# VodLM/vod

Hardware: AMD Instinct MI355X
Metric: queries/sec brute-force top-k (10Mx768 fp16) (higher is better)
Workload: dtype f16; 1 GPU; 10000000 sections x 768 f16, batch 1024 queries, top-100, exact brute force; rows_per_gpu=10000000, parallelism=single GPU, engine=ranks, recovery_passes=0

## Files before the change

### include/vodhip.h

```cpp
#ifndef VODHIP_H
#define VODHIP_H

#include <stdint.h>

#ifdef __cplusplus
extern "C" {
#endif

#define VODHIP_VERSION 1

enum { VODHIP_F16 = 0, VODHIP_BF16 = 1, VODHIP_F32 = 2 };
#define VODHIP_EXACT_F32 0x100
#define VODHIP_L2 0x200
enum { VODHIP_HOST = 0, VODHIP_DEVICE = 1 };

typedef struct vodhip_index vodhip_index_t;

const char* vodhip_last_error(void);
int vodhip_version(void);

int vodhip_index_create(int device, int64_t dim, int store_dtype ,
                        int64_t capacity_rows, vodhip_index_t** out);
int vodhip_index_destroy(vodhip_index_t* index);

// ... 47 lines not shown

#define VODHIP_POSTERIOR_GROUP_ROWS 16384
#define VODHIP_POSTERIOR_TEMP_BYTES (256ll << 20)
int vodhip_index_posterior_mean(vodhip_index_t* index, const void* queries, int q_dtype, int64_t nq, float beta,
                                const int32_t* q_labels_dev , int n_per_query,
                                float* out_max , float* out_log_rel ,
                                float* out_mean , void* stream);

#define VODHIP_SAMPLE_SLACK_TILES 2
int vodhip_index_sample_posterior(vodhip_index_t* index, const void* queries, int q_dtype, int64_t nq, int k, float beta, uint64_t seed,
                                  int64_t query_offset, int64_t id_base, const int32_t* q_labels_dev ,
                                  int n_per_query, float* out_max , float* out_log_rel ,
                                  int64_t* out_ids , float* out_scores, float* out_log_p,
                                  float* out_log_weight , float* out_keys , void* stream);

#define VODHIP_RANK_MAX_LISTED 64
int vodhip_index_count_above(vodhip_index_t* index, const void* queries, int q_dtype, int64_t nq, const float* thresholds_dev,
                             const int64_t* tie_ids_dev , int64_t m, int64_t id_base,
                             const int32_t* q_labels_dev , int n_per_query,
                             int64_t* out_counts , void* stream);
int vodhip_index_rank_ids(vodhip_index_t* index, const void* queries, int q_dtype, int64_t nq, const int64_t* ids_dev, int64_t m,
                          int64_t id_base, const int32_t* q_labels_dev , int n_per_query,
                          int64_t* out_ranks , float* out_scores , void* stream);
int vodhip_index_scan_score_ids(vodhip_index_t* index, const void* queries, int q_dtype, int64_t nq, const int64_t* ids_dev, int64_t m,
                                int64_t id_base, const int32_t* q_labels_dev , int n_per_query,
                                float* out_scores , int32_t* out_rows , void* stream);

int vodhip_index_set_row_labels(vodhip_index_t* index, const int32_t* labels, int64_t n_rows, int location, void* stream);
int vodhip_index_set_query_labels(vodhip_index_t* index, const int32_t* q_labels_dev, int n_per_query);

int vodhip_index_set_param(vodhip_index_t* index, const char* key, int64_t value);
int vodhip_debug_schedule(int64_t ntotal, int k, int64_t nq, int64_t cand_cap, int64_t dense_rows, int64_t sample_div,
                          int64_t growth_x100, int tile, int recovery_pass, int n_cu, int64_t* out, int max_stages);
int vodhip_index_get_stat(const vodhip_index_t* index, const char* key, int64_t* out);
int vodhip_debug_l2_split(float c, int dtype, uint16_t terms[3], float consts[3]);
int vodhip_debug_tile_order(int64_t ntotal, int64_t* perm_mul, int64_t* perm_mod);
int vodhip_debug_read_probe(int which, int64_t* out, int n);

int vodhip_merge_topk(const float* scores, const int64_t* ids, int n_shards, int64_t nq, int k,
                      int k_out, float* out_scores, int64_t* out_ids, void* stream);
int vodhip_merge_topk_strided(const float* scores, int64_t shard_stride_scores, const int64_t* ids,
                              int64_t shard_stride_ids, int n_shards, int64_t nq, int k, int k_out,
                              float* out_scores, int64_t* out_ids, void* stream);

typedef struct vodhip_node_index vodhip_node_index_t;
int vodhip_node_index_create(int n_devices, const int* devices, int64_t dim, int store_dtype, int64_t capacity_rows,
                             vodhip_node_index_t** out);
int vodhip_node_index_destroy(vodhip_node_index_t* index);
int vodhip_node_index_add(vodhip_node_index_t* index, const void* rows, int64_t n_rows, int src_dtype);
int vodhip_node_index_reset(vodhip_node_index_t* index);
int vodhip_node_index_ntotal(const vodhip_node_index_t* index, int64_t* out);
int vodhip_node_index_n_shards(const vodhip_node_index_t* index);
int vodhip_node_index_shard(vodhip_node_index_t* index, int g, vodhip_index_t** shard, int64_t* id_base, int* device);
int vodhip_node_index_set_param(vodhip_node_index_t* index, const char* key, int64_t value);
int vodhip_node_index_peer_access(const vodhip_node_index_t* index, int* out, int n);
int vodhip_node_index_set_row_labels(vodhip_node_index_t* index, const int32_t* labels, int64_t n_rows);
int vodhip_node_index_set_query_labels(vodhip_node_index_t* index, const int32_t* q_labels, int n_per_query, int location);
int vodhip_node_index_search(vodhip_node_index_t* index, const void* queries, int q_dtype, int64_t nq, int k, int location,
                             float* out_scores, int64_t* out_ids, void* stream);
int vodhip_node_index_search_async(vodhip_node_index_t* index, const void* queries, int q_dtype, int64_t nq, int k, int location,
                                   float* out_scores, int64_t* out_ids, void* stream);
int vodhip_node_index_search_finish(vodhip_node_index_t* index);
int vodhip_node_index_score_ids(vodhip_node_index_t* index, const void* queries, int q_dtype, int64_t nq, const int64_t* ids, int64_t m,
                                const int32_t* q_labels, int n_per_query, int location, float* out_scores, void* stream);
int vodhip_node_index_search_ids(vodhip_node_index_t* index, const void* queries, int q_dtype, int64_t nq, const int64_t* ids, int64_t m,
                                 int k, const int32_t* q_labels, int n_per_query, int location, float* out_scores, int64_t* out_ids,
// ... 248 lines not shown
```

### vod_amd/_native.py

```python
from __future__ import annotations

import ctypes
import pathlib
import threading

_LIB_NAME = "libvodhip.so"
_lock = threading.Lock()
_lib: ctypes.CDLL | None = None

F16, BF16, F32 = 0, 1, 2
EXACT_F32 = 0x100
L2 = 0x200
METRICS = {"inner_product": 0, "l2": L2}


def metric_flag(metric: str) -> int:
    if metric not in METRICS:
        raise ValueError(f"metric must be one of {sorted(METRICS)}, got {metric!r}")
    return METRICS[metric]
HOST, DEVICE = 0, 1
MAX_K = 2048
MAX_LISTED = 8192
MAX_ENGINES = 4

# ... 17 lines not shown
SIGNATURES: dict[str, tuple] = {
    "vodhip_last_error": (_c.c_char_p, []),
    "vodhip_version": (_i32, []),
    "vodhip_index_create": (_i32, [_i32, _i64, _i32, _i64, _c.POINTER(_vp)]),
    "vodhip_index_destroy": (_i32, [_vp]),
    "vodhip_index_add": (_i32, [_vp, _vp, _i64, _i32, _i32, _vp]),
    "vodhip_index_reset": (_i32, [_vp]),
    "vodhip_index_ntotal": (_i32, [_vp, _c.POINTER(_i64)]),
    "vodhip_index_dim": (_i32, [_vp, _c.POINTER(_i64)]),
    "vodhip_index_capacity": (_i32, [_vp, _c.POINTER(_i64)]),
    "vodhip_index_data": (_i32, [_vp, _c.POINTER(_vp), _c.POINTER(_i64), _c.POINTER(_i32)]),
    "vodhip_index_get_rows": (_i32, [_vp, _i64, _i64, _vp, _i32, _vp]),
    "vodhip_index_data_f32": (_i32, [_vp, _c.POINTER(_vp), _c.POINTER(_i64)]),
    "vodhip_index_get_rows_f32": (_i32, [_vp, _i64, _i64, _vp, _i32, _vp]),
    "vodhip_index_search": (_i32, [_vp, _vp, _i32, _i64, _i32, _i64, _vp, _vp, _vp]),
    "vodhip_index_search_async": (_i32, [_vp, _vp, _i32, _i64, _i32, _i64, _vp, _vp, _vp]),
    "vodhip_index_search_finish": (_i32, [_vp, _vp]),
    "vodhip_index_score_ids": (_i32, [_vp, _vp, _i32, _i64, _vp, _i64, _i64, _vp, _i32, _vp, _vp]),
    "vodhip_index_search_ids": (_i32, [_vp, _vp, _i32, _i64, _vp, _i64, _i32, _i64, _vp, _i32, _vp, _vp, _vp]),
    "vodhip_index_sum_ids": (_i32, [_vp, _vp, _vp, _i64, _i64, _i64, _vp, _i32, _vp, _vp]),
    "vodhip_index_log_partition": (_i32, [_vp, _vp, _i32, _i64, _c.c_float, _vp, _i32, _vp, _vp, _vp]),
    "vodhip_index_posterior_stats": (_i32, [_vp, _vp, _i32, _i64, _c.c_float, _vp, _i32, _vp, _vp, _vp, _vp, _vp]),
    "vodhip_index_posterior_divergence": (_i32, [_vp, _vp, _vp, _i32, _i64, _c.c_float, _c.c_float, _vp, _i32] + [_vp] * 8 + [_vp]),
    "vodhip_index_posterior_mean": (_i32, [_vp, _vp, _i32, _i64, _c.c_float, _vp, _i32, _vp, _vp, _vp, _vp]),
    "vodhip_index_count_above": (_i32, [_vp, _vp, _i32, _i64, _vp, _vp, _i64, _i64, _vp, _i32, _vp, _vp]),
    "vodhip_index_rank_ids": (_i32, [_vp, _vp, _i32, _i64, _vp, _i64, _i64, _vp, _i32, _vp, _vp, _vp]),
    "vodhip_index_scan_score_ids": (_i32, [_vp, _vp, _i32, _i64, _vp, _i64, _i64, _vp, _i32, _vp, _vp, _vp]),
    "vodhip_index_sample_posterior": (
        _i32, [_vp, _vp, _i32, _i64, _i32, _c.c_float, _c.c_uint64, _i64, _i64, _vp, _i32, _vp, _vp, _vp, _vp, _vp, _vp, _vp, _vp]),
    "vodhip_index_set_row_labels": (_i32, [_vp, _vp, _i64, _i32, _vp]),
    "vodhip_index_set_query_labels": (_i32, [_vp, _vp, _i32]),
    "vodhip_index_set_param": (_i32, [_vp, _c.c_char_p, _i64]),
    "vodhip_debug_schedule": (_i32, [_i64, _i32, _i64, _i64, _i64, _i64, _i64, _i32, _i32, _i32, _c.POINTER(_i64), _i32]),
    "vodhip_index_get_stat": (_i32, [_vp, _c.c_char_p, _c.POINTER(_i64)]),
    "vodhip_debug_l2_split": (_i32, [_c.c_float, _i32, _c.POINTER(_c.c_uint16), _c.POINTER(_c.c_float)]),
    "vodhip_debug_tile_order": (_i32, [_i64, _c.POINTER(_i64), _c.POINTER(_i64)]),
    "vodhip_debug_read_probe": (_i32, [_i32, _c.POINTER(_i64), _i32]),
    "vodhip_node_index_create": (_i32, [_i32, _c.POINTER(_i32), _i64, _i32, _i64, _c.POINTER(_vp)]),
    "vodhip_node_index_destroy": (_i32, [_vp]),
    "vodhip_node_index_add": (_i32, [_vp, _vp, _i64, _i32]),
    "vodhip_node_index_reset": (_i32, [_vp]),
    "vodhip_node_index_ntotal": (_i32, [_vp, _c.POINTER(_i64)]),
    "vodhip_node_index_n_shards": (_i32, [_vp]),
    "vodhip_node_index_shard": (_i32, [_vp, _i32, _c.POINTER(_vp), _c.POINTER(_i64), _c.POINTER(_i32)]),
    "vodhip_node_index_set_param": (_i32, [_vp, _c.c_char_p, _i64]),
    "vodhip_node_index_get_stat": (_i32, [_vp, _c.c_char_p, _c.POINTER(_i64)]),
    "vodhip_node_index_peer_access": (_i32, [_vp, _c.POINTER(_i32), _i32]),
    "vodhip_node_index_set_row_labels": (_i32, [_vp, _vp, _i64]),
    "vodhip_node_index_set_query_labels": (_i32, [_vp, _vp, _i32, _i32]),
    "vodhip_node_index_search": (_i32, [_vp, _vp, _i32, _i64, _i32, _i32, _vp, _vp, _vp]),
    "vodhip_node_index_search_async": (_i32, [_vp, _vp, _i32, _i64, _i32, _i32, _vp, _vp, _vp]),
    "vodhip_node_index_search_finish": (_i32, [_vp]),
    "vodhip_node_index_score_ids": (_i32, [_vp, _vp, _i32, _i64, _vp, _i64, _vp, _i32, _i32, _vp, _vp]),
    "vodhip_node_index_search_ids": (_i32, [_vp, _vp, _i32, _i64, _vp, _i64, _i32, _vp, _i32, _i32, _vp, _vp, _vp]),
    "vodhip_node_index_sum_ids": (_i32, [_vp, _vp, _vp, _i64, _i64, _vp, _i32, _i32, _vp, _vp]),
    "vodhip_node_index_log_partition": (_i32, [_vp, _vp, _i32, _i64, _c.c_float, _vp, _i32, _vp, _vp]),
    "vodhip_node_index_posterior_stats": (_i32, [_vp, _vp, _i32, _i64, _c.c_float, _vp, _i32, _vp, _vp, _vp, _vp]),
    "vodhip_node_index_posterior_divergence": (_i32, [_vp, _vp, _vp, _i32, _i64, _c.c_float, _c.c_float, _vp, _i32] + [_vp] * 8),
    "vodhip_node_index_posterior_mean": (_i32, [_vp, _vp, _i32, _i64, _c.c_float, _vp, _i32, _vp, _vp, _vp]),
    "vodhip_node_index_rank_ids": (_i32, [_vp, _vp, _i32, _i64, _vp, _i64, _vp, _i32, _vp, _vp]),
    "vodhip_node_index_count_above": (_i32, [_vp, _vp, _i32, _i64, _vp, _vp, _i64, _vp, _i32, _vp]),
    "vodhip_node_index_sample_posterior": (
        _i32, [_vp, _vp, _i32, _i64, _i32, _c.c_float, _c.c_uint64, _i64, _vp, _i32, _vp, _vp, _vp, _vp, _vp, _vp, _vp]),
    "vodhip_merge_topk": (_i32, [_vp, _vp, _i32, _i64, _i32, _i32, _vp, _vp, _vp]),
    "vodhip_merge_topk_strided": (_i32, [_vp, _i64, _vp, _i64, _i32, _i64, _i32, _i32, _vp, _vp, _vp]),
    "vodhip_merge_hybrid": (
# ... 172 lines not shown
```

### vod_amd/csrc/kernels_mips_8phase.hip

```cpp
#include <hip/hip_runtime.h>

#include <type_traits>

#include "mips_common.h"

namespace vodhip {

namespace {
constexpr int P8_HALF = 128 * 128;
constexpr int P8_OPERANDS = 8 * P8_HALF;
constexpr int P8_WL_CAP = 256;
constexpr int P8_WL_FLUSH = 176;
constexpr int P8_TRANSPOSE_MAX_LANES = 2;
constexpr int P8_XPOSE = 8 * 2 * 32 * 4;
constexpr int P8_DRAIN_RECORDS = 112;
constexpr int P8_SC1 = 16;
static_assert(P8_DRAIN_RECORDS % 8 == 0 && P8_DRAIN_RECORDS * 132 + 256 <= P8_OPERANDS / 8, "drain staging");
constexpr int P8_LDS = P8_OPERANDS + 8 * P8_WL_CAP * 12 + P8_XPOSE;
static_assert(P8_LDS <= 160 * 1024, "LDS budget");
}

template <int DT, bool SUBSET, bool KEEPB0, int LEAD = 7>
__global__ __launch_bounds__(512, 2) void mips_filter8ph_kernel(
    const uint16_t* __restrict__ X, const uint16_t* __restrict__ Q, int dim_pad, int row_begin, int row_end, int n_xtiles,
    int n_qtiles, int nq, const float* __restrict__ thr_s, const key_t64* __restrict__ thr_key, key_t64* __restrict__ cand,
    unsigned int* __restrict__ cnt, int cap, unsigned int* __restrict__ overflow, FilterExtra ex, float* __restrict__ ring, int ring_cap) {
    constexpr int BM = 256, BN = 256, WN = 4, NWAVES = 8, TM = 128, TN = 64, MB = TM / 16, NB16 = TN / 16, ROW_BYTES = 128;
    extern __shared__ __attribute__((aligned(16))) char smem[];
    const int bid = blockIdx.x;
    const int xcd = bid & 7, jj = bid >> 3;
    const int qt = jj % n_qtiles;
    const int xt0 = (jj / n_qtiles) * 8 + xcd;
    const int xt_step = (int)gridDim.x / n_qtiles;
    if (xt0 >= n_xtiles) return;
    const int n_my = (n_xtiles - 1 - xt0) / xt_step + 1;
    const int tid = threadIdx.x;
    const int lane = tid & 63;
    const int wave = __builtin_amdgcn_readfirstlane(tid >> 6);
    const int wm = wave / WN, wn = wave % WN;
    const int q0 = qt * BN;
    const int nk = dim_pad / 64;
    const size_t row_stride = (size_t)dim_pad * 2;

    const int st_row = lane >> 3, st_slot = lane & 7;
    int super_cur = ex.perm_mod > 0 ? filter_tile_row0(ex, row_begin, xt0, BM) / BM : 0;
    int super_epi = super_cur;
    const int perm_inc = ex.perm_mod > 0 ? (int)(((unsigned long long)xt_step * (unsigned long long)ex.perm_mul) % (unsigned long long)ex.perm_mod) : 0;
    const char* a_src[2];
    const char* b_src[2];
#pragma unroll
// ... 54 lines not shown
                        a_src[0] += step;
                        a_src[1] += step;
                    } else {
                        s_active = false;
                    }
                }
            }
        }
    };
    using K0 = std::integral_constant<int, 0>;
    using K1 = std::integral_constant<int, 1>;
    using K2 = std::integral_constant<int, 2>;
    using K3 = std::integral_constant<int, 3>;

    const int fr = lane & 15, fq = lane >> 4;
    const int swz = (fr >> 1) & 7;

    float thr[NB16];
#pragma unroll
    for (int j = 0; j < NB16; ++j) {
        const int q = q0 + wn * TN + j * 16 + fr;
        thr[j] = q < nq ? thr_s[q] : __builtin_inff();
    }
#pragma unroll
    for (int j = 0; j < NB16; ++j) asm volatile("" : "+v"(thr[j]));
    wait_vmcnt<0>();

    WaveSurvivorList<P8_WL_CAP, SUBSET> wl(smem + P8_OPERANDS, NWAVES, wave);
    const SurvivorOut out{thr_key, cand, cnt, cap, overflow, ex};
    auto wl_append = [&](bool p, key_t64 key, int q) { if (wl.append(p, key, q, out)) wait_vmcnt<0>(); };
    auto wl_flush = [&]() { wl.flush(out); wait_vmcnt<0>(); };
    float* const xpose = (float*)(smem + P8_OPERANDS + NWAVES * P8_WL_CAP * 12) + wave * 64;
    const size_t ring_wave = (size_t)bid * NWAVES + wave;
    float* const ring_w = ring + ring_wave * ring_cap * 32;
    unsigned* const ring_meta = (unsigned*)(ring + (size_t)gridDim.x * NWAVES * ring_cap * 32) + ring_wave * ring_cap;
    int ring_n = 0;
    int ring_fallbacks = 0;

    f32x4 acc[MB][NB16];
    u32x4 fa[4], fb[2], fa1[4], fb1[2];
    u32x4 fc[2], fc1[2];
#ifdef P8_KNOBS
    const bool knob_no_stagger = (ex.flags & (1 << 8)) != 0, knob_no_prio = (ex.flags & (2 << 8)) != 0;
#else
    constexpr bool knob_no_stagger = false, knob_no_prio = false;
#endif

    auto read_a = [&](const char* half) {
        const char* base = half + (wm * 64 + fr) * ROW_BYTES;
        const int s0 = ((0 + fq) ^ swz) << 4, s1 = ((4 + fq) ^ swz) << 4;
#pragma unroll
        for (int i = 0; i < 4; ++i) {
            fa[i] = *(const u32x4*)(base + i * 16 * ROW_BYTES + s0);
            fa1[i] = *(const u32x4*)(base + i * 16 * ROW_BYTES + s1);
        }
    };
    auto read_b = [&](const char* half) {
        const char* base = half + (wn * 32 + fr) * ROW_BYTES;
        const int s0 = ((0 + fq) ^ swz) << 4, s1 = ((4 + fq) ^ swz) << 4;
#pragma unroll
        for (int j = 0; j < 2; ++j) {
            fb[j] = *(const u32x4*)(base + j * 16 * ROW_BYTES + s0);
            fb1[j] = *(const u32x4*)(base + j * 16 * ROW_BYTES + s1);
        }
    };
    auto read_b1 = [&](const char* half) {
        const char* base = half + (wn * 32 + fr) * ROW_BYTES;
        const int s0 = ((0 + fq) ^ swz) << 4, s1 = ((4 + fq) ^ swz) << 4;
// ... 53 lines not shown
        for (int j = 0; j < NB16; ++j) {
            mj[j] = vmax3(acc[0][j][0], acc[0][j][1], acc[0][j][2]);
            mj[j] = fmaxf_raw(mj[j], acc[0][j][3]);
        }
#pragma unroll
        for (int i = 1; i < MB; ++i)
#pragma unroll
            for (int j = 0; j < NB16; ++j) {
                mj[j] = vmax3(mj[j], acc[i][j][0], acc[i][j][1]);
                mj[j] = vmax3(mj[j], acc[i][j][2], acc[i][j][3]);
            }
#ifdef P8_ABL_NO_EMIT
#pragma unroll
        for (int j = 0; j < NB16; ++j) {
            const unsigned long long any_hit = __ballot(mj[j] >= thr[j]);
            asm volatile("" ::"s"(any_hit));
        }
        (void)x0;
        return;
#else
        unsigned long long hl[NB16];
#pragma unroll
        for (int j = 0; j < NB16; ++j) hl[j] = __ballot(mj[j] >= thr[j]);
        if ((hl[0] | hl[1] | hl[2] | hl[3]) == 0ull) {
            if (wl.n >= P8_WL_FLUSH) wl_flush();
            return;
        }
        static_assert(NB16 == 4, "the early-out above");
#pragma unroll
        for (int j = 0; j < NB16; ++j) {
            const float m = mj[j];
            const bool hit = m >= thr[j];
            const unsigned long long hit_lanes = hl[j];
            if (hit_lanes != 0ull && ring_n + __builtin_popcountll(hit_lanes) <= ring_cap) {
                if (hit) {
                    const int slot = ring_n + (int)__builtin_amdgcn_mbcnt_hi((unsigned)(hit_lanes >> 32), __builtin_amdgcn_mbcnt_lo((unsigned)hit_lanes, 0u));
                    f32x4* const rec = (f32x4*)(ring_w + (size_t)slot * 32);
#pragma unroll
                    for (int i = 0; i < MB; ++i) rec[i] = acc[i][j];
                    int x0_o = x0, lane_o = lane;
                    asm volatile("" : "+s"(x0_o));
                    asm volatile("" : "+v"(lane_o));
                    ring_meta[slot] = (unsigned)x0_o | (unsigned)(j << 6) | (unsigned)lane_o;
                }
                ring_n += __builtin_popcountll(hit_lanes);
            } else if (hit_lanes != 0ull) {
                ++ring_fallbacks;
                int x0_o = x0, row_end_o = row_end, lane_o = lane;
                asm volatile("" : "+s"(x0_o), "+s"(row_end_o));
                asm volatile("" : "+v"(lane_o));
                auto transpose_emit = [&](unsigned long long src_lanes, bool mine) __attribute__((always_inline)) {
                    const int rank = (int)__builtin_amdgcn_mbcnt_hi((unsigned)(src_lanes >> 32), __builtin_amdgcn_mbcnt_lo((unsigned)src_lanes, 0u));
                    const int half = lane_o >> 5, t = lane_o & 31;
                    unsigned long long rest = src_lanes;
                    int done = 0;
                    do {
                        const int slot = rank - done;
                        if (mine && (unsigned)slot < 2u) {
                            float* dst = xpose + slot * 32;
#pragma unroll
                            for (int i = 0; i < MB; ++i) *(f32x4*)(dst + 4 * i) = acc[i][j];
                        }
                        wave_lds_exchange();
                        const int l0 = __builtin_ctzll(rest);
                        rest &= rest - 1ull;
                        const bool two = rest != 0ull;
                        const int l1 = two ? __builtin_ctzll(rest) : l0;
                        rest &= rest - 1ull;
                        const float t0 = __builtin_bit_cast(float, __builtin_amdgcn_readlane(__builtin_bit_cast(int, thr[j]), l0));
                        const float t1 = __builtin_bit_cast(float, __builtin_amdgcn_readlane(__builtin_bit_cast(int, thr[j]), l1));
                        const float sc = xpose[lane_o];
                        const int src = half ? l1 : l0;
                        const float thr_src = half ? t1 : t0;
                        const int q_src = q0 + wn * TN + j * 16 + (src & 15);
                        const int rw = x0_o + wm * TM + 4 * (src >> 4) + (t >> 2) * 16 + (t & 3);
                        wl_append((half == 0 || two) && sc >= thr_src && rw < row_end_o, make_key(sc, (unsigned)rw), q_src);
                        done += 2;
                        wave_lds_exchange();
                    } while (rest != 0ull);
// ... 62 lines not shown
            read_a(kb + 2 * P8_HALF);
            stage(S2{});
            asm volatile("s_waitcnt lgkmcnt(0)" ::: "memory");
            __builtin_amdgcn_s_barrier();
            if (first) mma_quadrant(1, 1, true); else mma_quadrant(1, 1, false);
            __builtin_amdgcn_s_barrier();
            if constexpr (!KEEPB0) read_b(kb + 3 * P8_HALF);
            stage(S3{});
            wait_next_ktile(kt + 1);
            asm volatile("s_waitcnt lgkmcnt(0)" ::: "memory");
            __builtin_amdgcn_s_barrier();
            if (first) mma_quadrant(1, 0, true); else mma_quadrant(1, 0, false);
            __builtin_amdgcn_s_barrier();
        }
        epilogue(x0);
        if (ex.perm_mod > 0) {
            int nxt = super_epi + perm_inc;
            if (nxt >= ex.perm_mod) nxt -= ex.perm_mod;
            super_epi = nxt;
        }
    }
    if (wm == 0 && !knob_no_stagger) __builtin_amdgcn_s_barrier();

#ifndef P8_ABL_NO_DRAIN
    if (ring_n > 0) {
        wait_vmcnt<0>();
        if (fq == 0) {
#pragma unroll
            for (int j = 0; j < NB16; ++j) xpose[j * 16 + fr] = thr[j];
        }
        wave_lds_exchange();
        char* const stage_w = smem + wave * (P8_OPERANDS / NWAVES);
        const float* const sums = (const float*)stage_w;
        const unsigned* const meta = (const unsigned*)(stage_w + P8_DRAIN_RECORDS * 128);
        const int half = lane >> 5, t = lane & 31;
        for (int r0 = 0; r0 < ring_n; r0 += P8_DRAIN_RECORDS) {
#pragma unroll
            for (int i = 0; i < P8_DRAIN_RECORDS / 8; ++i) {
                const int r = min(r0 + i * 8 + (lane >> 3), ring_n - 1);
                __builtin_amdgcn_global_load_lds((const VOD_AS1 void*)(ring_w + (size_t)r * 32 + (lane & 7) * 4),
                                                 (VOD_AS3 void*)(stage_w + i * 1024), 16, 0, P8_SC1);
            }
#pragma unroll
            for (int i = 0; i < (P8_DRAIN_RECORDS + 63) / 64; ++i) {
                const int r = min(r0 + i * 64 + lane, ring_n - 1);
                __builtin_amdgcn_global_load_lds((const VOD_AS1 void*)(ring_meta + r), (VOD_AS3 void*)(stage_w + P8_DRAIN_RECORDS * 128 + i * 256),
                                                 4, 0, P8_SC1);
            }
            wait_vmcnt<0>();
            const int nr = min(ring_n - r0, P8_DRAIN_RECORDS);
            for (int r4 = 0; r4 < nr; r4 += 4) {
                if (wl.n > P8_WL_CAP - 128) wl_flush();
                const int r = r4 + half;
#pragma unroll
                for (int u = 0; u < 4; u += 2) {
                    const float v = sums[(r + u) * 32 + t];
                    const unsigned m = meta[r + u];
                    const int src = (int)(m & 63u), jb = (int)((m >> 6) & 3u), x0 = (int)(m & ~255u);
                    const int q_src = q0 + wn * TN + jb * 16 + (src & 15);
                    const int rw = x0 + wm * TM + 4 * (src >> 4) + (t >> 2) * 16 + (t & 3);
                    wl_append(r + u < nr && v >= xpose[jb * 16 + (src & 15)] && rw < row_end, make_key(v, (unsigned)rw), q_src);
                }
            }
        }
    }
#endif
    wl_flush();
    if (ring_fallbacks > 0 && lane == 0) atomicAdd(overflow + 3, (unsigned)ring_fallbacks);
}

template <bool KEEPB0, int LEAD = 7>
static hipError_t launch_8phase(int store_dtype, const void* store, const void* q_pad, int64_t dim_pad, int64_t row_begin, int64_t row_end, int n_xtiles,
                                   int64_t nq, int64_t nq_pad, const SearchWorkspace& ws, hipStream_t stream) {
    const bool subset = ws.extra.row_label != nullptr;
    const int n_qtiles = (int)(nq_pad / 256);
    const int n_cu = ws.n_cu > 0 ? ws.n_cu : 256;
    const int unit = 8 * n_qtiles;
    const int total = ((n_xtiles + 7) / 8) * unit;
    int grid = (n_cu / unit) * unit;
    if (grid < unit) grid = unit;
    if (grid > total) grid = total;
    const int ring_cap = ws.ring ? (int)std::min<int64_t>(ws.ring_cap, ws.ring_floats / ((int64_t)grid * 8 * 33)) : 0;
    auto launch = [&](auto kern) -> hipError_t {
        if (hipError_t e = allow_dynamic_lds((const void*)kern, P8_LDS); e != hipSuccess) return e;
        hipLaunchKernelGGL(kern, dim3((unsigned)grid), dim3(512), P8_LDS, stream, (const uint16_t*)store, (const uint16_t*)q_pad, (int)dim_pad,
                           (int)row_begin, (int)row_end, n_xtiles, n_qtiles, (int)nq, ws.thr_s, ws.thr_key, ws.cand, ws.cnt, (int)ws.cap,
                           ws.overflow, ws.extra, ws.ring, ring_cap);
        return hipGetLastError();
    };
    if constexpr (LEAD != 7)
        return store_dtype == 0 ? launch(mips_filter8ph_kernel<0, false, KEEPB0, LEAD>) : launch(mips_filter8ph_kernel<1, false, KEEPB0, LEAD>);
    else if (subset) return store_dtype == 0 ? launch(mips_filter8ph_kernel<0, true, KEEPB0>) : launch(mips_filter8ph_kernel<1, true, KEEPB0>);
    else return store_dtype == 0 ? launch(mips_filter8ph_kernel<0, false, KEEPB0>) : launch(mips_filter8ph_kernel<1, false, KEEPB0>);
}

hipError_t launch_filter_8phase(int store_dtype, int lead, bool keep_b0, const void* store, const void* q_pad, int64_t dim_pad, int64_t row_begin,
                                int64_t row_end, int64_t nq, int64_t nq_pad, const SearchWorkspace& ws, hipStream_t stream) {
    constexpr FilterGeometry G = geometry(FilterKernel::EightPhase);
    static_assert(G.rows == 256 && G.cols == 256 && G.persistent, "the planner's geometry of mips_filter8ph_kernel");
    int n_xtiles = (int)((row_end - row_begin + 255) / 256);
    if (ws.extra.perm_mod > 0) row_end = ws.extra.row_bound;
#ifdef VODHIP_EXPERIMENTS
    if (lead == 6) return launch_8phase<true, 6>(store_dtype, store, q_pad, dim_pad, row_begin, row_end, n_xtiles, nq, nq_pad, ws, stream);
    if (lead == 5) return launch_8phase<true, 5>(store_dtype, store, q_pad, dim_pad, row_begin, row_end, n_xtiles, nq, nq_pad, ws, stream);
    if (!keep_b0) return launch_8phase<false>(store_dtype, store, q_pad, dim_pad, row_begin, row_end, n_xtiles, nq, nq_pad, ws, stream);
#endif
    (void)lead;
    (void)keep_b0;
    return launch_8phase<true>(store_dtype, store, q_pad, dim_pad, row_begin, row_end, n_xtiles, nq, nq_pad, ws, stream);
}

}
```

### vod_amd/csrc/search_plan.cpp

```cpp
#include "search_plan.h"

#include <stdint.h>

#include <algorithm>

namespace vodhip {

namespace {

void make_safe_schedule(int64_t n, int64_t cap, std::vector<Stage>& st) {
    const int64_t step = std::max<int64_t>(ROW_ALIGN, cap / ROW_ALIGN * ROW_ALIGN);
    for (int64_t b = 0; b < n; b += step) st.push_back({ST_DENSE, b, std::min(n, b + step), 0, 0, 0});
}

void make_geometric_schedule(int64_t n, int k, int64_t cap, std::vector<Stage>& st) {
    int64_t b = std::min(n, std::max<int64_t>(ROW_ALIGN, std::min<int64_t>(cap, 2048) / ROW_ALIGN * ROW_ALIGN));
    if (b < k && b < n) return make_safe_schedule(n, cap, st);
    st.push_back({ST_DENSE, 0, b, 0, 0, 0});
    const double growth = std::min(8.0, std::max(1.25, 1.0 + (double)cap / (4.0 * k)));
    while (b < n) {
        const int64_t e = std::min(n, round_up(std::max((int64_t)((double)b * growth), b + ROW_ALIGN), ROW_ALIGN));
        st.push_back({ST_FILTER, b, e, 0, 0, 0});
        b = e;
    }
// ... 61 lines not shown

SearchPlan plan_search(int64_t ntotal, int k, int64_t nq, const PlanTunables& t, bool subset, bool safe, int recovery) {
    SearchPlan p;
    const FilterKernel base = t.tile != 0 ? (FilterKernel)t.tile
                                          : nq > 128 ? FilterKernel::Persistent : (nq > 64 ? FilterKernel::Generic256x128 : FilterKernel::Generic256x64);
    const FilterGeometry& g = geometry(base);
    p.bn = g.cols;
    const int64_t nq_pad = round_up(std::min(MAX_NQ_PER_PASS, nq), p.bn);
    std::vector<Stage>& st = p.stages;
    if (subset && !safe && recovery == 0) make_geometric_schedule(ntotal, k, t.cand_cap, st);
    else make_schedule(ntotal, k, t, g, nq_pad, safe, recovery, st);
    p.corpus_nt = g.persistent && nq_pad == 256;
    bool all_filter = !st.empty();
    for (const Stage& sg : st) all_filter = all_filter && (sg.kind == ST_FILTER || sg.kind == ST_GMAX);
    const int64_t T = (ntotal + ROW_ALIGN - 1) / ROW_ALIGN;
    if (all_filter && t.tile_order == 0 && T >= 8) {
        const int64_t P = tile_order_multiplier(T);
        if (P > 1) {
            p.perm_mul = P;
            p.perm_mod = T;
        }
    }
    const bool auto_8phase = t.tile == 0 && nq > 128 && !subset;
    if (t.tile == 0 && g.persistent) p.small_tiles = t.small_chunk_tiles;
    for (Stage& sg : st) {
        sg.kernel = base;
        if (sg.kind == ST_DENSE && g.persistent) sg.kernel = FilterKernel::Generic128;
        if (sg.kind == ST_GMAX && base == FilterKernel::EightPhase) sg.kernel = FilterKernel::Persistent;
        if (sg.kind == ST_FILTER && auto_8phase) sg.kernel = FilterKernel::EightPhase;
        if (sg.kind == ST_GMAX) sg.sample_offset = ((ntotal - 1) - (sg.n_tiles * geometry(sg.kernel).rows - 1) * sg.rstride) / 2;
    }
    double per_query = 0.0;
    int64_t calibrated = ntotal;
    for (const Stage& sg : st) {
        if (sg.kind == ST_GMAX) calibrated = sg.n_tiles * geometry(sg.kernel).rows;
        if (sg.kind == ST_FILTER && sg.kernel == FilterKernel::EightPhase)
            per_query = std::max(per_query, 1.4 * k * (double)(sg.e - sg.b) / (double)std::max<int64_t>(1, calibrated));
        if (sg.kind != ST_GMAX) calibrated = sg.e;
    }
    if (per_query > 0.0) p.ring = t.survivor_ring > 0 ? t.survivor_ring : survivor_ring_records(per_query, nq_pad, t.n_cu);
    return p;
}

int64_t survivor_ring_records(double per_query, int64_t nq_pad, int n_cu) {
    const int64_t n_qt = std::max<int64_t>(1, nq_pad / 256);
    const int64_t unit = 8 * n_qt;
    const int64_t grid = std::max(unit, std::max(1, n_cu) / unit * unit);
    const double per_wave = per_query * 64.0 / (double)(2 * grid / n_qt);
    return std::min<int64_t>(MAX_AUTO_SURVIVOR_RING, round_up((int64_t)(2.0 * per_wave) + 64, 64));
}

int64_t tile_order_multiplier(int64_t T) {
    if (T < 8) return 0;
    const int64_t P0 = (int64_t)((double)T * 0.6180339887498949);
    int64_t best = 0, best_q = INT64_MAX;
    for (int64_t d = 0; d <= 64; ++d) {
        for (int sgn = 0; sgn < 2; ++sgn) {
            const int64_t P = sgn ? P0 - d : P0 + d;
            if (P <= 1 || P >= T || (d == 0 && sgn)) continue;
            int64_t a = T, b = P, worst = 0;
            bool first = true;
            while (b) {
                const int64_t quo = a / b, rem = a % b;
                if (!first) worst = std::max(worst, quo);
                first = false;
                a = b;
                b = rem;
            }
            if (a != 1) continue;
            if (worst < best_q) {
                best_q = worst;
                best = P;
            }
        }
    }
    return best;
}

}
```

### vod_amd/csrc/search_plan.h

```cpp
#pragma once
#include <stdint.h>

#include <vector>

namespace vodhip {

inline int64_t round_up(int64_t v, int64_t m) { return (v + m - 1) / m * m; }

constexpr int64_t ROW_ALIGN = 256;
constexpr int64_t MAX_NQ_PER_PASS = 2048;
constexpr int64_t MAX_SURVIVOR_RING = 8192;
constexpr int64_t MAX_AUTO_SURVIVOR_RING = 1024;

enum class FilterKernel : int { Generic128 = 1, Generic256x64 = 42, Generic256x128 = 46, Persistent = 8, Staggered = 9, EightPhase = 14 };

struct FilterGeometry {
    FilterKernel kernel;
    int rows, cols;
    int group_rows;
    bool persistent;
};
constexpr FilterGeometry FILTER_KERNELS[] = {
    {FilterKernel::Generic128, 128, 128, 16, false},
    {FilterKernel::Generic256x64, 256, 64, 16, false},
    {FilterKernel::Generic256x128, 256, 128, 16, false},
    {FilterKernel::Persistent, 256, 256, 32, true},
    {FilterKernel::Staggered, 256, 256, 32, true},
    {FilterKernel::EightPhase, 256, 256, 32, true},
};
constexpr const FilterGeometry* find_kernel(int64_t id) {
    for (const FilterGeometry& g : FILTER_KERNELS)
        if ((int64_t)g.kernel == id) return &g;
    return nullptr;
}
constexpr const FilterGeometry& geometry(FilterKernel f) { return *find_kernel((int64_t)f); }

enum : int { ST_FILTER = 0, ST_DENSE = 1, ST_GMAX = 2 };
struct Stage {
    int kind;
    int64_t b, e;
    int64_t n_tiles;
    int64_t rstride;
    int64_t n_groups;
    FilterKernel kernel = FilterKernel::Persistent;
    int64_t sample_offset = 0;
};

struct PlanTunables {
    int64_t cand_cap = 16384;
    int64_t dense_rows = 2048;
    int64_t growth_x100 = 0;
    int64_t sample_div = 0;
    int64_t tile = 0;
    int64_t tile_order = 0;
    int64_t small_chunk_tiles = 256;
    int64_t survivor_ring = 0;
    int n_cu = 256;
};

struct SearchPlan {
    int64_t bn = 256;
    bool corpus_nt = false;
    int64_t perm_mul = 0, perm_mod = 0;
    int64_t small_tiles = 0;
    std::vector<Stage> stages;
    int64_t ring = 0;
    FilterKernel kernel(const Stage& sg, int64_t nq_pad) const {
        return sg.kind == ST_FILTER && (sg.e - sg.b + 255) / 256 * (nq_pad / 256) < small_tiles ? FilterKernel::Generic128 : sg.kernel;
    }
};

SearchPlan plan_search(int64_t ntotal, int k, int64_t nq, const PlanTunables& t, bool subset, bool safe, int recovery);

int64_t survivor_ring_records(double per_query, int64_t nq_pad, int n_cu);

int64_t tile_order_multiplier(int64_t T);

}
```

### vod_amd/csrc/vodhip_api.hip

```cpp
#include "../../include/vodhip.h"

#include <algorithm>
#include <atomic>
#include <cmath>
#include <cstdarg>
#include <cstdio>
#include <cstdint>
#include <cstring>
#include <string>
#include <deque>
#include <initializer_list>
#include <mutex>
#include <thread>
#include <vector>

#include "l2_bias.h"
#include "partition_fold.h"
#include "sample_fold.h"
#include "rank_fold.h"
#include "stats_fold.h"
#include "divergence_fold.h"
#include "search_plan.h"
#include "vodhip_internal.h"

// ... 144 lines not shown
    (void)hipFree(w.overflow);
    (void)hipFree(w.ring);
    const int n_cu = w.n_cu;
    w = SearchWorkspace();
    w.n_cu = n_cu;
    return 0;
}

int ensure_workspace(vodhip_index* ix, int lane, int64_t nq_pad, int64_t cap, int64_t kp) {
    SearchWorkspace& w = ix->ws_lane[lane];
    if (w.nq_cap >= nq_pad && w.cap == cap && w.kp_cap >= kp && w.q_pad) {
        w.kp = kp;
        return 0;
    }
    const int64_t nq_cap = std::max(nq_pad, w.nq_cap);
    const int64_t kp_cap = std::max(kp, w.kp_cap);
    free_workspace(ix, lane);
    HIP_OK(hipMalloc((void**)&w.q_pad, (size_t)nq_cap * ix->dim_pad * 2));
    HIP_OK(hipMalloc((void**)&w.topk, (size_t)nq_cap * kp_cap * sizeof(key_t64)));
    HIP_OK(hipMalloc((void**)&w.cand, (size_t)nq_cap * cap * sizeof(key_t64)));
    HIP_OK(hipMalloc((void**)&w.cnt, (size_t)nq_cap * CNT_STRIDE * sizeof(unsigned int)));
    HIP_OK(hipMalloc((void**)&w.thr_s, (size_t)nq_cap * sizeof(float)));
    HIP_OK(hipMalloc((void**)&w.thr_key, (size_t)nq_cap * sizeof(key_t64)));
    HIP_OK(hipMalloc((void**)&w.overflow, FLAG_WORDS * sizeof(unsigned int)));
    w.nq_cap = nq_cap;
    w.cap = cap;
    w.kp = kp;
    w.kp_cap = kp_cap;
    return 0;
}

int ensure_ring(vodhip_index* ix, int lane, int64_t records) {
    SearchWorkspace& w = ix->ws_lane[lane];
    const int64_t floats = (int64_t)std::max(w.n_cu, 64) * 8 * records * 33;
    if (floats > w.ring_floats) {
        (void)hipFree(w.ring);
        w.ring = nullptr;
        w.ring_floats = 0;
        if (hipMalloc((void**)&w.ring, (size_t)floats * sizeof(float)) != hipSuccess) {
            (void)hipGetLastError();
            w.ring = nullptr;
            w.ring_cap = 0;
            return 0;
        }
        w.ring_floats = floats;
    }
    w.ring_cap = records;
    return 0;
}

void exact_bound_args(const vodhip_index* ix, ExactArgs& xa) {
    xa.ord_n2 = ix->ord_n2;
    xa.ord_d2 = ix->ord_d2;
    xa.cut_n2 = ix->cut_n2;
    xa.cut_d2 = ix->cut_d2;
    xa.n_out = ix->n_out;
    xa.out_rows = ix->norm_stats + EXS_OUT_ROWS;
    xa.row_n2 = ix->row_n2;
    xa.row_d2 = ix->row_d2;
}

int refresh_exact_stats(vodhip_index* ix, hipStream_t stream) {
    if (!ix->exact || !ix->stats_dirty) return 0;
    HIP_OK(launch_exact_stats(ix->row_n2, ix->row_d2, ix->ntotal, ix->norm_stats, stream));
    unsigned int w[8];
    HIP_OK(hipMemcpyAsync(w, ix->norm_stats, sizeof(w), hipMemcpyDeviceToHost, stream));
    HIP_OK(hipStreamSynchronize(stream));
// ... 1241 lines not shown
    for (int i = 0; i < 6; ++i)
        if (ev[i]) (void)hipEventDestroy(ev[i]);
    if (le != hipSuccess) return fail("sample-posterior launch failed: %s", hipGetErrorString(le));
    HIP_OK(se);
    ix->last_sample[0] = st[0];
    ix->last_sample[1] = st[1];
    ix->last_sample[2] = st[2];
    ix->last_sample[3] = st[3];
    ix->last_sample[4] = (int64_t)(((uint64_t)st[5] << 32) | st[4]);
    ix->last_sample[5] = emit_groups;
    for (int i = 0; i < 5; ++i) ix->last_sample_ns[i] = (int64_t)ns[i];
    if (st[0]) return fail("candidate list overflow: %u queries met more than %d tile maxima tied with their threshold", st[0], VODHIP_SAMPLE_SLACK_TILES);
    return 0;
}

int vodhip_debug_schedule(int64_t ntotal, int k, int64_t nq, int64_t cand_cap, int64_t dense_rows, int64_t sample_div,
                          int64_t growth_x100, int tile, int recovery_pass, int n_cu, int64_t* out, int max_stages) {
    PlanTunables t;
    if (cand_cap > 0) t.cand_cap = cand_cap;
    if (dense_rows > 0) t.dense_rows = round_up(dense_rows, ROW_ALIGN);
    if (sample_div > 0) t.sample_div = sample_div;
    t.growth_x100 = growth_x100;
    t.tile = tile;
    if (n_cu > 0) t.n_cu = n_cu;
    if (!out || max_stages < 1 || k < 1 || nq < 1 || ntotal < 0 || (tile != 0 && !find_kernel(tile) && !experiment_filter(t)))
        return fail("invalid arguments");
    const std::vector<Stage> st = plan_search(ntotal, k, nq, t, false, false, recovery_pass).stages;
    if ((int)st.size() > max_stages) return fail("%d stages do not fit max_stages=%d", (int)st.size(), max_stages);
    for (size_t i = 0; i < st.size(); ++i) {
        const int64_t row[6] = {st[i].kind, st[i].b, st[i].e, st[i].n_tiles, st[i].rstride, st[i].n_groups};
        memcpy(out + i * 6, row, sizeof(row));
    }
    return (int)st.size();
}

int vodhip_debug_tile_order(int64_t ntotal, int64_t* perm_mul, int64_t* perm_mod) {
    if (!perm_mul || !perm_mod || ntotal < 0) return fail("invalid arguments");
    *perm_mod = (ntotal + ROW_ALIGN - 1) / ROW_ALIGN;
    *perm_mul = tile_order_multiplier(*perm_mod);
    return 0;
}

int vodhip_index_set_param(vodhip_index_t* ix, const char* key, int64_t value) {
    if (!ix || !key) return fail("NULL argument");
    if (!strcmp(key, "cand_cap")) {
        if (value < ROW_ALIGN || value > (1 << 16)) return fail("cand_cap must be in [256, 65536]");
        ix->tune.cand_cap = value;
    } else if (!strcmp(key, "dense_rows")) {
        if (value < ROW_ALIGN) return fail("dense_rows must be >= 256");
        ix->tune.dense_rows = round_up(value, ROW_ALIGN);
    } else if (!strcmp(key, "growth")) {
        ix->tune.growth_x100 = value;
    } else if (!strcmp(key, "force_safe")) {
        ix->force_safe = value;
    } else if (!strcmp(key, "small_chunk_tiles")) {
        ix->tune.small_chunk_tiles = value;
    } else if (!strcmp(key, "kflags")) {
        ix->kflags = value;
    } else if (!strcmp(key, "sample_div")) {
        if (value != 0 && value < 2) return fail("sample_div must be 0 (auto) or >= 2");
        ix->tune.sample_div = value;
    } else if (!strcmp(key, "profile")) {
        ix->profile = value;
    } else if (!strcmp(key, "ingest_threads")) {
        if (value < 0 || value > 256) return fail("ingest_threads must be in [0, 256] (0 = auto)");
        ix->ingest_threads = value;
// ... 719 lines not shown
```

Before: 83170 queries/s.

## Store survivor ring records per 16-row block instead of full accumulator columns

The survivor ring in the eight-phase filter kernel now stores only the 4-float accumulator sub-blocks whose max passes the threshold, along with packed metadata that includes the sub-block index. Previously each surviving lane wrote a full 32-float column. Ring memory per record drops from 33 to 5 floats, and the drain stage reads compact 16-byte records in larger batches. Ring sizing now accounts for workgroup count versus tile count, and the ring is disabled when rows exceed 2^29, since the metadata packing cannot address more. The cost is extra ballots and max computations per hit and a more complex per-sub-block append path.

```diff
diff --git a/include/vodhip.h b/include/vodhip.h
--- a/include/vodhip.h
+++ b/include/vodhip.h
@@ -103,6 +103,7 @@
 int vodhip_index_set_param(vodhip_index_t* index, const char* key, int64_t value);
 int vodhip_debug_schedule(int64_t ntotal, int k, int64_t nq, int64_t cand_cap, int64_t dense_rows, int64_t sample_div,
                           int64_t growth_x100, int tile, int recovery_pass, int n_cu, int64_t* out, int max_stages);
+int vodhip_debug_survivor_ring(int64_t ntotal, int k, int64_t nq, int tile, int64_t survivor_ring, int n_cu, int64_t* records);
 int vodhip_index_get_stat(const vodhip_index_t* index, const char* key, int64_t* out);
 int vodhip_debug_l2_split(float c, int dtype, uint16_t terms[3], float consts[3]);
 int vodhip_debug_tile_order(int64_t ntotal, int64_t* perm_mul, int64_t* perm_mod);
diff --git a/vod_amd/_native.py b/vod_amd/_native.py
--- a/vod_amd/_native.py
+++ b/vod_amd/_native.py
@@ -73,6 +73,7 @@
     "vodhip_index_set_query_labels": (_i32, [_vp, _vp, _i32]),
     "vodhip_index_set_param": (_i32, [_vp, _c.c_char_p, _i64]),
     "vodhip_debug_schedule": (_i32, [_i64, _i32, _i64, _i64, _i64, _i64, _i64, _i32, _i32, _i32, _c.POINTER(_i64), _i32]),
+    "vodhip_debug_survivor_ring": (_i32, [_i64, _i32, _i64, _i32, _i64, _i32, _c.POINTER(_i64)]),
     "vodhip_index_get_stat": (_i32, [_vp, _c.c_char_p, _c.POINTER(_i64)]),
     "vodhip_debug_l2_split": (_i32, [_c.c_float, _i32, _c.POINTER(_c.c_uint16), _c.POINTER(_c.c_float)]),
     "vodhip_debug_tile_order": (_i32, [_i64, _c.POINTER(_i64), _c.POINTER(_i64)]),
diff --git a/vod_amd/csrc/kernels_mips_8phase.hip b/vod_amd/csrc/kernels_mips_8phase.hip
--- a/vod_amd/csrc/kernels_mips_8phase.hip
+++ b/vod_amd/csrc/kernels_mips_8phase.hip
@@ -13,9 +13,9 @@
 constexpr int P8_WL_FLUSH = 176;
 constexpr int P8_TRANSPOSE_MAX_LANES = 2;
 constexpr int P8_XPOSE = 8 * 2 * 32 * 4;
-constexpr int P8_DRAIN_RECORDS = 112;
+constexpr int P8_DRAIN_RECORDS = 768;
 constexpr int P8_SC1 = 16;
-static_assert(P8_DRAIN_RECORDS % 8 == 0 && P8_DRAIN_RECORDS * 132 + 256 <= P8_OPERANDS / 8, "drain staging");
+static_assert(P8_DRAIN_RECORDS % 64 == 0 && P8_DRAIN_RECORDS * RING_RECORD_BYTES <= P8_OPERANDS / 8, "drain staging");
 constexpr int P8_LDS = P8_OPERANDS + 8 * P8_WL_CAP * 12 + P8_XPOSE;
 static_assert(P8_LDS <= 160 * 1024, "LDS budget");
 }
@@ -136,8 +136,8 @@
     auto wl_flush = [&]() { wl.flush(out); wait_vmcnt<0>(); };
     float* const xpose = (float*)(smem + P8_OPERANDS + NWAVES * P8_WL_CAP * 12) + wave * 64;
     const size_t ring_wave = (size_t)bid * NWAVES + wave;
-    float* const ring_w = ring + ring_wave * ring_cap * 32;
-    unsigned* const ring_meta = (unsigned*)(ring + (size_t)gridDim.x * NWAVES * ring_cap * 32) + ring_wave * ring_cap;
+    f32x4* const ring_w = (f32x4*)ring + ring_wave * ring_cap;
+    unsigned* const ring_meta = (unsigned*)(ring + (size_t)gridDim.x * NWAVES * ring_cap * 4) + ring_wave * ring_cap;
     int ring_n = 0;
     int ring_fallbacks = 0;
 
@@ -257,19 +257,37 @@
             const float m = mj[j];
             const bool hit = m >= thr[j];
             const unsigned long long hit_lanes = hl[j];
-            if (hit_lanes != 0ull && ring_n + __builtin_popcountll(hit_lanes) <= ring_cap) {
-                if (hit) {
-                    const int slot = ring_n + (int)__builtin_amdgcn_mbcnt_hi((unsigned)(hit_lanes >> 32), __builtin_amdgcn_mbcnt_lo((unsigned)hit_lanes, 0u));
-                    f32x4* const rec = (f32x4*)(ring_w + (size_t)slot * 32);
-#pragma unroll
-                    for (int i = 0; i < MB; ++i) rec[i] = acc[i][j];
+            bool in_loop = hit_lanes != 0ull;
+            if (in_loop && ring_n < ring_cap) {
+                bool hb[MB];
+                unsigned long long hbl[MB];
+                int records = 0;
+#pragma unroll
+                for (int i = 0; i < MB; ++i) {
+                    hb[i] = fmaxf_raw(vmax3(acc[i][j][0], acc[i][j][1], acc[i][j][2]), acc[i][j][3]) >= thr[j];
+                    hbl[i] = __ballot(hb[i]);
+                    records += __builtin_popcountll(hbl[i]);
+                }
+                if (ring_n + records <= ring_cap) {
+                    in_loop = false;
                     int x0_o = x0, lane_o = lane;
                     asm volatile("" : "+s"(x0_o));
                     asm volatile("" : "+v"(lane_o));
-                    ring_meta[slot] = (unsigned)x0_o | (unsigned)(j << 6) | (unsigned)lane_o;
-                }
-                ring_n += __builtin_popcountll(hit_lanes);
-            } else if (hit_lanes != 0ull) {
+                    const unsigned meta = ((unsigned)x0_o << 3) | (unsigned)(j << 6) | (unsigned)lane_o;
+#pragma unroll
+                    for (int i = 0; i < MB; ++i) {
+                        if (hbl[i] != 0ull) {
+                            if (hb[i]) {
+                                const int slot = ring_n + (int)__builtin_amdgcn_mbcnt_hi((unsigned)(hbl[i] >> 32), __builtin_amdgcn_mbcnt_lo((unsigned)hbl[i], 0u));
+                                ring_w[slot] = acc[i][j];
+                                ring_meta[slot] = meta | (unsigned)(i << 8);
+                            }
+                            ring_n += __builtin_popcountll(hbl[i]);
+                        }
+                    }
+                }
+            }
+            if (in_loop) {
                 ++ring_fallbacks;
                 int x0_o = x0, row_end_o = row_end, lane_o = lane;
                 asm volatile("" : "+s"(x0_o), "+s"(row_end_o));
@@ -398,34 +416,27 @@
         wave_lds_exchange();
         char* const stage_w = smem + wave * (P8_OPERANDS / NWAVES);
         const float* const sums = (const float*)stage_w;
-        const unsigned* const meta = (const unsigned*)(stage_w + P8_DRAIN_RECORDS * 128);
-        const int half = lane >> 5, t = lane & 31;
+        const unsigned* const meta = (const unsigned*)(stage_w + P8_DRAIN_RECORDS * 16);
         for (int r0 = 0; r0 < ring_n; r0 += P8_DRAIN_RECORDS) {
-#pragma unroll
-            for (int i = 0; i < P8_DRAIN_RECORDS / 8; ++i) {
-                const int r = min(r0 + i * 8 + (lane >> 3), ring_n - 1);
-                __builtin_amdgcn_global_load_lds((const VOD_AS1 void*)(ring_w + (size_t)r * 32 + (lane & 7) * 4),
-                                                 (VOD_AS3 void*)(stage_w + i * 1024), 16, 0, P8_SC1);
-            }
-#pragma unroll
-            for (int i = 0; i < (P8_DRAIN_RECORDS + 63) / 64; ++i) {
+            const int nr = min(ring_n - r0, P8_DRAIN_RECORDS);
+            for (int i = 0; i * 64 < nr; ++i) {
                 const int r = min(r0 + i * 64 + lane, ring_n - 1);
-                __builtin_amdgcn_global_load_lds((const VOD_AS1 void*)(ring_meta + r), (VOD_AS3 void*)(stage_w + P8_DRAIN_RECORDS * 128 + i * 256),
+                __builtin_amdgcn_global_load_lds((const VOD_AS1 void*)(ring_w + r), (VOD_AS3 void*)(stage_w + i * 1024), 16, 0, P8_SC1);
+                __builtin_amdgcn_global_load_lds((const VOD_AS1 void*)(ring_meta + r), (VOD_AS3 void*)(stage_w + P8_DRAIN_RECORDS * 16 + i * 256),
                                                  4, 0, P8_SC1);
             }
             wait_vmcnt<0>();
-            const int nr = min(ring_n - r0, P8_DRAIN_RECORDS);
-            for (int r4 = 0; r4 < nr; r4 += 4) {
+            for (int r32 = 0; r32 < nr; r32 += 32) {
                 if (wl.n > P8_WL_CAP - 128) wl_flush();
-                const int r = r4 + half;
-#pragma unroll
-                for (int u = 0; u < 4; u += 2) {
-                    const float v = sums[(r + u) * 32 + t];
-                    const unsigned m = meta[r + u];
-                    const int src = (int)(m & 63u), jb = (int)((m >> 6) & 3u), x0 = (int)(m & ~255u);
+#pragma unroll
+                for (int u = 0; u < 2; ++u) {
+                    const int r = r32 + u * 16 + (lane >> 2);
+                    const float v = sums[r * 4 + (lane & 3)];
+                    const unsigned m = meta[r];
+                    const int src = (int)(m & 63u), jb = (int)((m >> 6) & 3u), ib = (int)((m >> 8) & 7u), x0 = (int)((m >> 11) << 8);
                     const int q_src = q0 + wn * TN + jb * 16 + (src & 15);
-                    const int rw = x0 + wm * TM + 4 * (src >> 4) + (t >> 2) * 16 + (t & 3);
-                    wl_append(r + u < nr && v >= xpose[jb * 16 + (src & 15)] && rw < row_end, make_key(v, (unsigned)rw), q_src);
+                    const int rw = x0 + wm * TM + 4 * (src >> 4) + ib * 16 + (lane & 3);
+                    wl_append(r < nr && v >= xpose[jb * 16 + (src & 15)] && rw < row_end, make_key(v, (unsigned)rw), q_src);
                 }
             }
         }
@@ -446,7 +457,8 @@
     int grid = (n_cu / unit) * unit;
     if (grid < unit) grid = unit;
     if (grid > total) grid = total;
-    const int ring_cap = ws.ring ? (int)std::min<int64_t>(ws.ring_cap, ws.ring_floats / ((int64_t)grid * 8 * 33)) : 0;
+    const bool ring_rows_ok = round_up(row_end, 256) <= RING_MAX_ROWS;
+    const int ring_cap = ws.ring && ring_rows_ok ? (int)std::min<int64_t>(ws.ring_cap, ws.ring_floats / ((int64_t)grid * 8 * RING_RECORD_FLOATS)) : 0;
     auto launch = [&](auto kern) -> hipError_t {
         if (hipError_t e = allow_dynamic_lds((const void*)kern, P8_LDS); e != hipSuccess) return e;
         hipLaunchKernelGGL(kern, dim3((unsigned)grid), dim3(512), P8_LDS, stream, (const uint16_t*)store, (const uint16_t*)q_pad, (int)dim_pad,
diff --git a/vod_amd/csrc/search_plan.cpp b/vod_amd/csrc/search_plan.cpp
--- a/vod_amd/csrc/search_plan.cpp
+++ b/vod_amd/csrc/search_plan.cpp
@@ -117,21 +117,29 @@
     }
     double per_query = 0.0;
     int64_t calibrated = ntotal;
+    const double wgs = (double)survivor_ring_workgroups(nq_pad, t.n_cu);
     for (const Stage& sg : st) {
         if (sg.kind == ST_GMAX) calibrated = sg.n_tiles * geometry(sg.kernel).rows;
-        if (sg.kind == ST_FILTER && sg.kernel == FilterKernel::EightPhase)
-            per_query = std::max(per_query, 1.4 * k * (double)(sg.e - sg.b) / (double)std::max<int64_t>(1, calibrated));
+        if (sg.kind == ST_FILTER && sg.kernel == FilterKernel::EightPhase) {
+            const double tiles = (double)((sg.e - sg.b + 255) / 256);
+            per_query = std::max(per_query, 1.4 * k * (double)(sg.e - sg.b) / (double)std::max<int64_t>(1, calibrated) * std::max(1.0, wgs / tiles));
+        }
         if (sg.kind != ST_GMAX) calibrated = sg.e;
     }
-    if (per_query > 0.0) p.ring = t.survivor_ring > 0 ? t.survivor_ring : survivor_ring_records(per_query, nq_pad, t.n_cu);
+    if (per_query > 0.0 && round_up(ntotal, ROW_ALIGN) <= RING_MAX_ROWS)
+        p.ring = t.survivor_ring > 0 ? t.survivor_ring : survivor_ring_records(per_query, nq_pad, t.n_cu);
     return p;
 }
 
-int64_t survivor_ring_records(double per_query, int64_t nq_pad, int n_cu) {
+int64_t survivor_ring_workgroups(int64_t nq_pad, int n_cu) {
     const int64_t n_qt = std::max<int64_t>(1, nq_pad / 256);
     const int64_t unit = 8 * n_qt;
     const int64_t grid = std::max(unit, std::max(1, n_cu) / unit * unit);
-    const double per_wave = per_query * 64.0 / (double)(2 * grid / n_qt);
+    return grid / n_qt;
+}
+
+int64_t survivor_ring_records(double per_query, int64_t nq_pad, int n_cu) {
+    const double per_wave = per_query * 64.0 / (double)(2 * survivor_ring_workgroups(nq_pad, n_cu));
     return std::min<int64_t>(MAX_AUTO_SURVIVOR_RING, round_up((int64_t)(2.0 * per_wave) + 64, 64));
 }
 
diff --git a/vod_amd/csrc/search_plan.h b/vod_amd/csrc/search_plan.h
--- a/vod_amd/csrc/search_plan.h
+++ b/vod_amd/csrc/search_plan.h
@@ -10,6 +10,9 @@
 constexpr int64_t ROW_ALIGN = 256;
 constexpr int64_t MAX_NQ_PER_PASS = 2048;
 constexpr int64_t MAX_SURVIVOR_RING = 8192;
+constexpr int64_t RING_RECORD_FLOATS = 5;
+constexpr int64_t RING_RECORD_BYTES = 4 * RING_RECORD_FLOATS;
+constexpr int64_t RING_MAX_ROWS = 1ll << 29;
 constexpr int64_t MAX_AUTO_SURVIVOR_RING = 1024;
 
 enum class FilterKernel : int { Generic128 = 1, Generic256x64 = 42, Generic256x128 = 46, Persistent = 8, Staggered = 9, EightPhase = 14 };
@@ -73,6 +76,7 @@
 SearchPlan plan_search(int64_t ntotal, int k, int64_t nq, const PlanTunables& t, bool subset, bool safe, int recovery);
 
 int64_t survivor_ring_records(double per_query, int64_t nq_pad, int n_cu);
+int64_t survivor_ring_workgroups(int64_t nq_pad, int n_cu);
 
 int64_t tile_order_multiplier(int64_t T);
 
diff --git a/vod_amd/csrc/vodhip_api.hip b/vod_amd/csrc/vodhip_api.hip
--- a/vod_amd/csrc/vodhip_api.hip
+++ b/vod_amd/csrc/vodhip_api.hip
@@ -200,7 +200,7 @@
 
 int ensure_ring(vodhip_index* ix, int lane, int64_t records) {
     SearchWorkspace& w = ix->ws_lane[lane];
-    const int64_t floats = (int64_t)std::max(w.n_cu, 64) * 8 * records * 33;
+    const int64_t floats = (int64_t)std::max(w.n_cu, 64) * 8 * records * RING_RECORD_FLOATS;
     if (floats > w.ring_floats) {
         (void)hipFree(w.ring);
         w.ring = nullptr;
@@ -1508,6 +1508,17 @@
         memcpy(out + i * 6, row, sizeof(row));
     }
     return (int)st.size();
+}
+
+int vodhip_debug_survivor_ring(int64_t ntotal, int k, int64_t nq, int tile, int64_t survivor_ring, int n_cu, int64_t* records) {
+    PlanTunables t;
+    t.tile = tile;
+    t.survivor_ring = survivor_ring;
+    if (n_cu > 0) t.n_cu = n_cu;
+    if (!records || k < 1 || nq < 1 || ntotal < 0 || survivor_ring < 0 || survivor_ring > MAX_SURVIVOR_RING || (tile != 0 && !find_kernel(tile)))
+        return fail("invalid arguments");
+    *records = plan_search(ntotal, k, nq, t, false, false, 0).ring;
+    return 0;
 }
 
 int vodhip_debug_tile_order(int64_t ntotal, int64_t* perm_mul, int64_t* perm_mod) {
```

New measurement: 83610 queries/s, median of 6. About the same (+0.5%).
